# CHONSPQX/modulated-deform-conv

Hardware: AMD Instinct MI355X
Metric: fwd+bwd GSamples/s, MDCN2d 3x3 C=256 56x56 B=32; %HBM roofline (higher is better)
Workload: dtype f32; 1 GPU; ModulatedDeformConv2d 3x3, C_in=C_out=256, 56x56, deformable_group=1, fp32, B=32 per GPU, forward+backward (BASELINE.json configs[1]); global_batch=32, parallelism=dp1 batch-sharded

## Files before the change

### modulated_deform_conv_amd/csrc/mfma_bwd_data.hip

```cpp
#include "mfma_kernels.hpp"
#include "mfma_tile.hpp"
#include <algorithm>
#include <map>
#include <mutex>
#include <stdio.h>
#include <stdlib.h>

namespace mdconv {

namespace {

int grid_for(int64_t total) {
  int64_t b = (total + 255) / 256;
  return (int)(b > 8192 ? 8192 : (b < 1 ? 1 : b));
}

__device__ __forceinline__ void pack_wq_items(const Geom &g, int ochunks, int cblks, const float *__restrict__ w,
                                              float *__restrict__ wq, int64_t first, int64_t step) {
  const int64_t total = (int64_t)g.K * ochunks * cblks * 2 * 64;
  for (int64_t i = first; i < total; i += step) {
    int64_t r = i;
    const int lane = (int)(r & 63); r >>= 6;
    const int q = (int)(r & 1); r >>= 1;
    const int cblk = (int)(r % cblks); r /= cblks;
// ... 6 lines not shown
    for (int s = 0; s < 4; ++s) {
      const int o = ob + s;
      v[s] = (o < g.O && c < g.C && o / g.Og == c / g.Cg)
                 ? w[((int64_t)o * g.Cg + (c % g.Cg)) * g.K + tap] : 0.f;
    }
    reinterpret_cast<float4 *>(wq)[i] = make_float4(v[0], v[1], v[2], v[3]);
  }
}

__global__ __launch_bounds__(256) void pack_wq_kernel(Geom g, int ochunks, int cblks,
                                                      const float *__restrict__ w,
                                                      float *__restrict__ wq) {
  pack_wq_items(g, ochunks, cblks, w, wq, (int64_t)blockIdx.x * 256 + threadIdx.x, (int64_t)gridDim.x * 256);
}

__global__ __launch_bounds__(256) void bwd_prep_kernel(Geom g, int ochunks, int cblks, const float *__restrict__ w,
                                                       float *__restrict__ wq, int *__restrict__ cnt, int64_t cnt_n,
                                                       const float *__restrict__ x, float *__restrict__ xt,
                                                       int nb_pack, int nb_zero, int qtiles, int ctiles) {
  __shared__ float t[32][33];
  int bid = blockIdx.x;
  if (bid < nb_pack) {
    pack_wq_items(g, ochunks, cblks, w, wq, (int64_t)bid * 256 + threadIdx.x, (int64_t)nb_pack * 256);
    return;
  }
  bid -= nb_pack;
  if (bid < nb_zero) {
    for (int64_t i = (int64_t)bid * 256 + threadIdx.x; i < cnt_n; i += (int64_t)nb_zero * 256) cnt[i] = 0;
    return;
  }
  bid -= nb_zero;
  const int qx = bid % qtiles, cy = (bid / qtiles) % ctiles, b = bid / (qtiles * ctiles);
  nchw_to_nhwc_tile(t, g.C, g.S_i, x, xt, b, cy * 32, qx * 32);
}



template <int ND, bool MOD, int WAVES_C, int QPQ, bool CL>
__global__ __launch_bounds__(256, 2) void mfma_bwd_data_kernel(
    Geom g, BwdDims bd, const float *__restrict__ input, const float *__restrict__ gout,
    const float *__restrict__ wq, const float *__restrict__ offset, const float *__restrict__ mask,
    float *__restrict__ gcol, float *__restrict__ grad_offset, float *__restrict__ grad_mask,
    float *__restrict__ ga, float *__restrict__ bias_part, int *__restrict__ cnt,
    int *__restrict__ table, const float *__restrict__ xt, int ntiles, int n_full, int n_tail, int tpw) {
  constexpr int NC = 1 << ND, NP = NC / 2;
  constexpr int MB = 2;
  constexpr int WAVES_P = 4 / WAVES_C;
  constexpr int BNP = 32 * WAVES_P;
  constexpr int RB = ND == 2 ? 8 : 4;
  constexpr int NBATCH = MB * 16 / RB;
  constexpr int HS = NBATCH / 2, CPS = NC / HS;
  constexpr int kOob = 0x7ffffff0;
  extern __shared__ __attribute__((aligned(16))) float smem[];
  const int T_o = bd.ochunks;
  const int gpitch = T_o * 16 + 4;
  float *Gs = smem;
  float *red = smem + BNP * gpitch;
  const int kTapGroup = bd.tap_group;

  const int tid = threadIdx.x, lane = tid & 63, kh = lane >> 5;
  const int wave = __builtin_amdgcn_readfirstlane(tid >> 6);
  const int wc = wave / WAVES_P, wp = wave % WAVES_P;

  int u0, u1;
  if ((int)blockIdx.x < n_full) {
    u0 = xcd_remap(blockIdx.x, n_full) * g.K * tpw;
    u1 = u0 + g.K * tpw;
  } else {
    const int j = xcd_remap(blockIdx.x - n_full, n_tail);
    const int64_t tail_units = (int64_t)(ntiles - n_full * tpw) * g.K;
    u0 = n_full * tpw * g.K + (int)(tail_units * j / n_tail);
    u1 = n_full * tpw * g.K + (int)(tail_units * (j + 1) / n_tail);
  }
  if (u0 >= u1) return;

  const int passes = bd.cblks_q / (2 * WAVES_C);
  const int iters = (u1 - u0) * passes;
// ... 37 lines not shown
#pragma unroll
      for (int q = 0; q < 2; ++q)
        ra[i][q] = buf_load4(r_wq, a_lane + (i * 2 + q) * frag_bytes, soff);
  };
  float4 ra0[MB][2], ra1[MB][2], ra2[MB][2], ra3[MB][2];
  {
    int q_lo, q_n;
    krange(0, q_lo, q_n);
    a_cur = a_base(u0 % g.K, 0, q_lo);
    n_cur = 4;
    load_a(ra0, a_off(0));
    load_a(ra1, a_off(1));
    load_a(ra2, a_off(2));
  }

  struct Pix { int n0, b, pix; bool live; int oc[ND]; };
  auto pix_of_tile = [&](int tile, Pix &px) {
    px.n0 = tile * BNP;
    const int n_raw = px.n0 + wp * 32 + (lane & 31);
    px.live = n_raw < g.N;
    const int n_l = px.live ? n_raw : g.N - 1;
    px.b = n_l / g.S_o;
    px.pix = n_l - px.b * g.S_o;
    out_coords<ND>(g, px.pix, px.oc);
  };
  Pix pc, pp;
  pix_of_tile(u0 / g.K, pc);
  pp = pc;

  auto load_gout_tile = [&](int tile) {
    const int j = tid % BNP, osub = tid / BNP;
    constexpr int OSTEP = 256 / BNP;
    const int n_t = min(tile * BNP + j, g.N - 1);
    const int b_t = n_t / g.S_o, pix_t = n_t - b_t * g.S_o;
    const bool t_live = tile * BNP + j < g.N;
    const float *src = gout + ((int64_t)b_t * g.O) * g.S_o + pix_t;
    float *dst = Gs + j * gpitch;
    const int Opad = T_o * 16;
#pragma unroll 8
// ... 78 lines not shown
  for (int pi = 0; pi < NP; ++pi) voff[pi] = kOob;
#pragma unroll
  for (int ci = 0; ci < NC; ++ci) voffc[ci] = kOob;
#pragma unroll
  for (int ci = 0; ci < NC; ++ci) S[ci] = 0.f;
#pragma unroll
  for (int a = 0; a < ND; ++a) delta_n[a] = 0.f;
#pragma unroll
  for (int a = 0; a < ND - 1; ++a) fac.ol[a] = fac.oh[a] = fac.osl[a] = fac.osh[a] = 0.f;
  fac.xw = fac.yw = fac.xs = fac.ys = 0.f;
#pragma unroll
  for (int i = 0; i < MB; ++i)
#pragma unroll
    for (int r = 0; r < 16; ++r) accp[i][r] = 0.f;

  auto new_tap_state = [&](int tapp, int dgp, bool count) {
    int tcd[ND];
    tap_coords<ND>(g, tapp, tcd);
    TapCoef<ND, float> tc;
    make_tap<ND, float>(g, pp.oc, tcd, delta_n, true, tc);
    mg = (!g.range_gate || tc.inside) ? m_n : 0.f;
    int pidx[NP];
    float px[NP], py[NP];
    make_pairs<ND, float>(g, tc, 1.f, pidx, px, py);
    bool prx[NP], pry[NP];
    make_pairs_read<ND, float>(g, tc, prx, pry);
    if (ND == 3 && count && kh == 0 && pp.live) {
      SampleAnchor<ND> sa;
      sample_anchor<ND>(g, tc, 1.f, sa);
      if (sa.on) atomicAdd(cnt + ((int64_t)pp.b * g.DG + dgp) * bd.S_e + sa.qa, 1);
    }
    if (ND == 2 && count && kh == 0 && pp.live) {
      int aidx[NP];
      float ax[NP], ay[NP];
      make_pairs_f<ND, float>(g, tc, tc.wl, tc.wha, 1.f, aidx, ax, ay);
      int *cseg = cnt + ((int64_t)pp.b * g.DG + dgp) * g.S_i;
#pragma unroll
      for (int pi = 0; pi < NP; ++pi)
        if (ax[pi] != 0.f || ay[pi] != 0.f) atomicAdd(cseg + aidx[pi], 1);
    }
    if (count && kh == 0) {
      const int n = pp.n0 + wp * 32 + lane;
      if (n < bd.Np) {
        int *e = table + ((int64_t)(dgp * g.K + tapp) * bd.Np + n) * (2 * NC);
        int ev[2 * NC];
#pragma unroll
        for (int pi = 0; pi < NP; ++pi) {
          if (bd.cl) {
            ev[2 * pi] = pp.live && prx[pi] ? (pp.b * g.S_i + pidx[pi]) * g.C * 4 : kOob;
            ev[2 * pi + 1] = pp.live && pry[pi] ? (pp.b * g.S_i + pidx[pi] + 1) * g.C * 4 : kOob;
          } else {
            ev[pi] = !pp.live ? 0
                     : ((prx[pi] || pry[pi]) ? ((pp.b * g.C * g.S_i + pidx[pi]) * 4) | (pry[pi] && !prx[pi] ? 1 : 0) | (prx[pi] && !pry[pi] ? 2 : 0)
                                             : kOob);
            ev[NP + pi] = 0;
          }
          ev[NC + 2 * pi] = pp.live ? __float_as_int(px[pi] * m_n) : 0;
          ev[NC + 2 * pi + 1] = pp.live ? __float_as_int(py[pi] * m_n) : 0;
        }
#pragma unroll
        for (int q4 = 0; q4 < 2 * NC; q4 += 4)
          *reinterpret_cast<int4 *>(e + q4) = make_int4(ev[q4], ev[q4 + 1], ev[q4 + 2], ev[q4 + 3]);
      }
    }
#pragma unroll
    for (int pi = 0; pi < NP; ++pi) {
      voff[pi] = (prx[pi] || pry[pi]) ? (pp.b * g.C * g.S_i + pidx[pi] + 4 * kh * g.S_i) * 4 : kOob;
      if (!CL) {
        bad[2 * pi] = __ballot(pry[pi] && !prx[pi]);
        bad[2 * pi + 1] = __ballot(prx[pi] && !pry[pi]);
      }
      voffc[2 * pi] = prx[pi] ? (pp.b * g.S_i + pidx[pi]) * g.C * 4 + 16 * kh : kOob;
      voffc[2 * pi + 1] = pry[pi] ? (pp.b * g.S_i + pidx[pi] + 1) * g.C * 4 + 16 * kh : kOob;
    }
    {
      constexpr int L = ND - 1;
      const int lc = tc.last_lc, hc = tc.last_lc + tc.delta[L];
      const int cl = min(lc, g.in_sz[L] - 2);
      fac.xw = (lc == cl ? tc.wl[L] : 0.f) + (hc == cl ? tc.wh[L] : 0.f);
      fac.yw = (lc == cl + 1 ? tc.wl[L] : 0.f) + (hc == cl + 1 ? tc.wh[L] : 0.f);
      fac.xs = (lc == cl ? tc.sl[L] : 0.f) + (hc == cl ? tc.sh[L] : 0.f);
      fac.ys = (lc == cl + 1 ? tc.sl[L] : 0.f) + (hc == cl + 1 ? tc.sh[L] : 0.f);
#pragma unroll
      for (int a = 0; a < L; ++a) { fac.ol[a] = tc.wl[a]; fac.oh[a] = tc.wh[a]; fac.osl[a] = tc.sl[a]; fac.osh[a] = tc.sh[a]; }
    }
    gc_voff = pp.live ? ((((pp.b * g.K + tapp) * g.S_o + pp.pix) * g.C) + 4 * kh) * 4 : kOob;
    if (CL && kh == 0) {
      int *st = St + lane * kStRow;
#pragma unroll
      for (int c4 = 0; c4 < NC; c4 += 4)
        *reinterpret_cast<int4 *>(st + c4) = make_int4(voffc[c4], voffc[c4 + 1], voffc[c4 + 2], voffc[c4 + 3]);
      st[NC] = gc_voff;
    }
#pragma unroll
    for (int ci = 0; ci < NC; ++ci) S[ci] = 0.f;
  };

  struct Batch { float f[RB * NC]; };
  auto gather = [&](int q, int cbase_p, Batch &v) {
    const int mb = (q * RB) / 16, r0 = (q * RB) % 16;
    if (CL) {
// ... 130 lines not shown
      const int pix = lane & 31, swz = pk_swz(pix);
      float *dst = Pk + pix * 64;
#pragma unroll
      for (int i = 0; i < MB; ++i)
#pragma unroll
        for (int rq = 0; rq < 4; ++rq)
          *reinterpret_cast<float4 *>(dst + 4 * ((i * 8 + 2 * rq + kh) ^ swz)) =
              make_float4(acc[i][4 * rq], acc[i][4 * rq + 1], acc[i][4 * rq + 2], acc[i][4 * rq + 3]);
    } else {
#pragma unroll
      for (int i = 0; i < MB; ++i) accp[i] = acc[i];
    }
  };

  int grp_lo = (u0 % g.K) % kTapGroup;
  auto finish_tap = [&](int tapp, int blk, bool flush_ok, bool last) {
    float goff[ND], gm = 0.f;
    {
      constexpr int L = ND - 1;
      float Tw[NP], Ts[NP];
#pragma unroll
      for (int pi = 0; pi < NP; ++pi) {
        Tw[pi] = fmaf(fac.xw, S[2 * pi], fac.yw * S[2 * pi + 1]);
        Ts[pi] = fmaf(fac.xs, S[2 * pi], fac.ys * S[2 * pi + 1]);
      }
#pragma unroll
      for (int a = 0; a < ND; ++a) goff[a] = 0.f;
#pragma unroll
      for (int pi = 0; pi < NP; ++pi) {
        float ow = 1.f;
#pragma unroll
// ... 7 lines not shown
          for (int a2 = 0; a2 < L; ++a2) {
            const bool hi = (pi >> (L - 1 - a2)) & 1;
            od *= (a2 == a) ? (hi ? fac.osh[a2] : fac.osl[a2]) : (hi ? fac.oh[a2] : fac.ol[a2]);
          }
          goff[a] = fmaf(od, Tw[pi], goff[a]);
        }
      }
#pragma unroll
      for (int a = 0; a < ND; ++a) goff[a] *= mg;
    }
    if (!CL) {
#pragma unroll
      for (int a = 0; a < ND; ++a) goff[a] += __shfl_xor(goff[a], 32, 64);
      gm += __shfl_xor(gm, 32, 64);
    }
    if (bd.red_floats == 0) {
      if (kh == 0 && pp.live) {
        const int64_t ob = ((int64_t)pp.b * (ND * g.K) + ND * tapp) * g.S_o + pp.pix;
#pragma unroll
        for (int a = 0; a < ND; ++a) {
          float *dst = grad_offset + ob + (int64_t)a * g.S_o;
          *dst = g.acc_data ? *dst + goff[a] : goff[a];
        }
        if (MOD) {
          float *dst = grad_mask + ((int64_t)pp.b * g.K + tapp) * g.S_o + pp.pix;
          *dst = g.acc_data ? *dst + gm : gm;
        }
      }
      return;
    }
    const int slot = tapp % kTapGroup;
    if (kh == 0) {
      float *rp = red + ((slot * nblk + blk) * (ND + 1)) * BNP + wp * 32 + lane;
#pragma unroll
      for (int a = 0; a < ND; ++a) rp[a * BNP] = goff[a];
      rp[ND * BNP] = gm;
    }
    if (flush_ok && (slot == kTapGroup - 1 || tapp == g.K - 1 || last)) {
      __syncthreads();
      const int tap0 = tapp - slot;
      const int per_slot = g.DG * (ND + 1) * BNP;
      const int items = (slot + 1 - grp_lo) * per_slot;
      for (int x = tid; x < items; x += 256) {
        const int jj = x % BNP, a = (x / BNP) % (ND + 1), dgi = (x / (BNP * (ND + 1))) % g.DG;
        const int sl = grp_lo + x / per_slot;
        const int n = pp.n0 + jj;
        if (n < g.N && (MOD || a < ND)) {
          float sum = 0.f;
          for (int y = 0; y < bpd; ++y)
            sum += red[((sl * nblk + dgi * bpd + y) * (ND + 1) + a) * BNP + jj];
          const int b = n / g.S_o, pix = n - b * g.S_o, tp = tap0 + sl;
          const int64_t seg = (int64_t)b * g.DG + dgi;
          float *dst = a < ND ? grad_offset + (seg * (ND * g.K) + ND * tp + a) * g.S_o + pix
                              : grad_mask + (seg * g.K + tp) * g.S_o + pix;
          *dst = g.acc_data ? *dst + sum : sum;
        }
      }
      __syncthreads();
      grp_lo = 0;
    }
  };

  auto mma = [&](const float4 (&ra)[MB][2], const float *bp, bool fresh) {
    const float4 b0 = *reinterpret_cast<const float4 *>(bp);
    const float4 b1 = *reinterpret_cast<const float4 *>(bp + 8);
    const f32x16 zero = {0.f, 0.f, 0.f, 0.f, 0.f, 0.f, 0.f, 0.f, 0.f, 0.f, 0.f, 0.f, 0.f, 0.f, 0.f, 0.f};
#pragma unroll
    for (int q = 0; q < 2; ++q)
#pragma unroll
// ... 16 lines not shown
    __builtin_amdgcn_sched_barrier(0);
    mma(ra1, bq + (t + 1) * 16, false);
    load_a(ra1, a_off(t + 5));
    __builtin_amdgcn_sched_barrier(0);
    mma(ra2, bq + (t + 2) * 16, false);
    load_a(ra2, a_off(t + 6));
    __builtin_amdgcn_sched_barrier(0);
    mma(ra3, bq + (t + 3) * 16, false);
  };
  auto quad = [&](int t, bool fresh) { quad_head(t); quad_tail(t, fresh); };

  int tile_c = -1;
  int tapp = 0, passp = 0;
  int tile = u0 / g.K, tap = u0 - tile * g.K, pass = 0;
  for (int it = 0; it < iters; ++it) {
    if (it > 0 && (passp == 0 || per_block)) {
      const int blk = passp * WAVES_C + wc;
      if (per_block) new_tap_state(tapp, min(blk * 64, g.C - 1) / g.Cdg, blk % bpd == 0 && blk * 64 < g.C);
      else new_tap_state(tapp, 0, wc == 0);
    }
    if (tile != tile_c) {
      if (tile_c >= 0) __syncthreads();
      if (gout_vec) load_gout_tile_vec(tile);
      else load_gout_tile(tile);
      pix_of_tile(tile, pc);
      tile_c = tile;
      __syncthreads();
      if (tap == 0 && pass == 0) emit_ga(tile);
    }
    if (pass == 0 || per_block) {
      const int dg = per_block ? min((pass * WAVES_C + wc) * 64, g.C - 1) / g.Cdg : 0;
      const int64_t seg = (int64_t)pc.b * g.DG + dg;
      const int64_t ob = (seg * (ND * g.K) + ND * tap) * g.S_o + pc.pix;
#pragma unroll
      for (int a = 0; a < ND; ++a) delta_n[a] = offset[ob + (int64_t)a * g.S_o];
      if (MOD) m_n = mask[(seg * g.K + tap) * g.S_o + pc.pix];
    }
    int nq;
    {
      int q_lo, tn = tap, pn = pass + 1;
      krange(pass, q_lo, nq);
      a_cur = a_base(tap, pass, q_lo);
      n_cur = nq * 4;
      b_cur = q_lo * 64;
      if (pn == passes) { pn = 0; tn = tap + 1 == g.K ? 0 : tap + 1; }
      int q_lo2, nq2;
      krange(pn, q_lo2, nq2);
      a_nxt = a_base(tn, pn, q_lo2);
    }
    const int cbase_p = (passp * WAVES_C + wc) * 64;
    if (QPQ == 0) {
// ... 12 lines not shown
      __builtin_amdgcn_sched_barrier(0);
      if (QPQ > 0) {
        quad_tail(q * QPQ * 4, q == 0);
#pragma unroll
        for (int jq = 1; jq < QPQ; ++jq) quad((q * QPQ + jq) * 4, false);
      } else {
        for (int qd = nq * q / NBATCH; qd < nq * (q + 1) / NBATCH; ++qd) quad(qd * 4, false);
      }
      __builtin_amdgcn_sched_barrier(0);
      consume(q, cbase_p, v);
      asm volatile("" ::: "memory");
      __builtin_amdgcn_sched_barrier(0);
    }
    collect();
    if (it > 0 && (passp == passes - 1 || per_block))
      finish_tap(tapp, per_block ? passp * WAVES_C + wc : wc, passp == passes - 1, false);
    park();
    pp = pc;
    tapp = tap;
    passp = pass;
    if (++pass == passes) {
      pass = 0;
      if (++tap == g.K) { tap = 0; ++tile; }
    }
  }
  {
    if (passp == 0 || per_block) {
      const int blk = passp * WAVES_C + wc;
      if (per_block) new_tap_state(tapp, min(blk * 64, g.C - 1) / g.Cdg, blk % bpd == 0 && blk * 64 < g.C);
      else new_tap_state(tapp, 0, wc == 0);
    }
    const int cbase_p = (passp * WAVES_C + wc) * 64;
    static_assert(NBATCH % 2 == 0, "pairs of drain batches");
#pragma unroll
    for (int q = 0; q < NBATCH; q += 2) {
      Batch v0, v1;
      gather(q, cbase_p, v0);
      gather(q + 1, cbase_p, v1);
      asm volatile("" ::: "memory");
      __builtin_amdgcn_sched_barrier(0);
      consume(q, cbase_p, v0);
      consume(q + 1, cbase_p, v1);
      asm volatile("" ::: "memory");
      __builtin_amdgcn_sched_barrier(0);
    }
    collect();
    finish_tap(tapp, per_block ? passp * WAVES_C + wc : wc, true, true);
  }
}


template <int ND, bool MOD>
__global__ __launch_bounds__(256) void csr_fill_kernel(Geom g, const float *__restrict__ offset,
                                                       const float *__restrict__ mask,
                                                       int *__restrict__ cursor,
                                                       const int *__restrict__ rowptr,
                                                       int4 *__restrict__ entries) {
  constexpr int NP = 1 << (ND - 1);
  const int64_t total = (int64_t)g.B * g.DG * g.K * g.S_o;
  for (int64_t i = (int64_t)blockIdx.x * 256 + threadIdx.x; i < total; i += (int64_t)gridDim.x * 256) {
    const int pix = (int)(i % g.S_o);
    const int tap = (int)((i / g.S_o) % g.K);
// ... 31 lines not shown
__global__ __launch_bounds__(256) void csr_scan_kernel(int S, const int *__restrict__ cnt,
                                            int *__restrict__ rowptr) {
  csr_scan_chunk(S, cnt, rowptr);
}

}

int pack_wq_f32(const Geom &g, const BwdDims &bd, const float *weight, float *wq, hipStream_t stream) {
  const int64_t total = (int64_t)g.K * bd.ochunks * bd.cblks_q * 2 * 64;
  hipLaunchKernelGGL(pack_wq_kernel, dim3(grid_for(total)), dim3(256), 0, stream, g, bd.ochunks,
                     bd.cblks_q, weight, wq);
  return check_launch("pack_wq");
}

int bwd_prep_f32(const Geom &g, const BwdDims &bd, const float *weight, float *wq, int *cnt, const float *x,
                 float *xt, hipStream_t stream) {
  const int64_t pack_total = (int64_t)g.K * bd.ochunks * bd.cblks_q * 2 * 64;
  const int64_t cnt_n = (int64_t)g.B * g.DG * bd.S_e;
  int nb_pack = grid_for(pack_total), nb_zero = grid_for(cnt_n);
  if (nb_pack > 512) nb_pack = 512;
  if (nb_zero > 256) nb_zero = 256;
  const int qtiles = (g.S_i + 31) / 32, ctiles = g.C / 32;
  const int64_t nb_t = xt ? (int64_t)qtiles * ctiles * g.B : 0;
  if (nb_t + nb_pack + nb_zero > 0x7fffffff) {
    int rc = pack_wq_f32(g, bd, weight, wq, stream);
    if (!rc) rc = csr_zero_f32(g, bd, cnt, stream);
    if (!rc && xt) rc = nchw_to_nhwc_f32(g, x, xt, stream);
    return rc;
  }
  hipLaunchKernelGGL(bwd_prep_kernel, dim3((unsigned)(nb_pack + nb_zero + nb_t)), dim3(256), 0, stream, g, bd.ochunks,
                     bd.cblks_q, weight, wq, cnt, cnt_n, x, xt, nb_pack, nb_zero, qtiles, ctiles);
  return check_launch("bwd_prep");
}

int num_cus() {
  static int n = 0;
  if (n == 0) {
    int dev = 0, v = 0;
    if (hipGetDevice(&dev) == hipSuccess &&
        hipDeviceGetAttribute(&v, hipDeviceAttributeMultiprocessorCount, dev) == hipSuccess && v > 0)
      n = v;
    else
      n = 256;
  }
  return n;
}

size_t bwd_data_lds_bytes(const Geom &g, const BwdDims &bd) {
  const int bnp = 32 * (4 / bd.waves_c);
  const int passes = bd.cblks_q / (2 * bd.waves_c);
  const size_t red = (size_t)bd.red_floats;
  const size_t cl = bd.cl_drain ? (size_t)4 * 32 * 64 + (size_t)4 * 32 * (2 * (1 << g.nd) + 4) : 0;
  return ((size_t)bnp * (bd.ochunks * 16 + 4) + red + cl) * sizeof(float);
}

int mfma_bwd_data_f32(const Geom &g, const BwdDims &bd, const Tensors &t, const float *wq,
                      float *gcol, float *ga, float *bias_part, int *cnt, int *table,
                      const float *xt, hipStream_t stream) {
#define LAUNCH_BD_(ND, MOD, WC, QPQ, CL)                                                            \
  do {                                                                                          \
    const int bnp = 32 * (4 / WC);                                                              \
    const int ntiles = (g.N + bnp - 1) / bnp;                                                   \
    const size_t lds = bwd_data_lds_bytes(g, bd);                                               \
     \
     \
     \
     \
    static std::once_flag attr_once;                                                            \
    static hipError_t attr_err = hipSuccess;                                                    \
    std::call_once(attr_once, [] {                                                              \
      attr_err = hipFuncSetAttribute((const void *)mfma_bwd_data_kernel<ND, MOD, WC, QPQ, CL>,  \
                                     hipFuncAttributeMaxDynamicSharedMemorySize, (int)kBwdDataLdsCap); \
    });                                                                                         \
// ... 14 lines not shown
        it = occ_by_lds.emplace(lds, nq > 0 ? nq : (lds * 2 <= 160 * 1024 ? 2 : 1)).first;      \
      }                                                                                         \
      occ_q = it->second;                                                                       \
    }                                                                                           \
    const int slots = num_cus() * occ_q;                                                        \
    const int tpw = 2;                        \
    const int n_full = ntiles / (slots * tpw) * slots;                                          \
    static const bool debug_plan = getenv("MDCONV_DEBUG_PLAN") != nullptr;                      \
    if (debug_plan)                                                                             \
      fprintf(stderr, "[mdconv] GEMM-1 plan: %d tiles, %zu B LDS, %d resident per CU\n", ntiles, lds, occ_q); \
    const int n_tail = (int)std::min<int64_t>((int64_t)(ntiles - n_full * tpw) * g.K, slots);   \
    hipLaunchKernelGGL((mfma_bwd_data_kernel<ND, MOD, WC, QPQ, CL>), dim3(n_full + n_tail), \
                       dim3(256), lds, stream,                                                  \
                       g, bd, (const float *)t.input, (const float *)t.grad_output, wq,         \
                       (const float *)t.offset, (const float *)t.mask, gcol,                    \
                       (float *)t.grad_offset, (float *)t.grad_mask, ga, bias_part, cnt, table, xt,        \
                       ntiles, n_full, n_tail, tpw);                                            \
  } while (0)
                                                \
#define LAUNCH_BD(ND, MOD, WC, QPQ)                                                             \
  do {                                                                                          \
    if (xt != nullptr && bd.cl_drain) LAUNCH_BD_(ND, MOD, WC, QPQ, true);                       \
    else LAUNCH_BD_(ND, MOD, WC, QPQ, false);                                                   \
  } while (0)
#define LAUNCH_BD2(ND, MOD)                                                                     \
  do {                                                                                          \
    const int nbatch = ND == 2 ? 4 : 8, nquads = bd.ochunks / 4;                                \
                   \
    const int qpq = (ND == 2 && g.G == 1 && nquads % nbatch == 0 && nquads / nbatch <= 2) ? nquads / nbatch : 0; \
    if (bd.waves_c == 4) {                                                                      \
      if (ND == 2 && qpq == 1) LAUNCH_BD(ND, MOD, 4, (ND == 2 ? 1 : 0));                        \
// ... 38 lines not shown
```

### modulated_deform_conv_amd/csrc/mfma_kernels.hip

```cpp
#include "mfma_plan.hpp"

#include <stdio.h>
#include <stdlib.h>

#include <atomic>
#include <mutex>
#include <vector>

namespace mdconv {

namespace {

__global__ __launch_bounds__(256) void pack_weights_kernel(Geom g, PackDims pd,
                                                           const float *__restrict__ w,
                                                           float *__restrict__ wp,
                                                           float *__restrict__ wq) {
  const int64_t total = (int64_t)g.G * g.K * pd.Cgp * pd.Ogp;
  const int mblks = pd.Ogp / 32, cchunks = pd.Cgp / kBK;
  for (int64_t i = (int64_t)blockIdx.x * 256 + threadIdx.x; i < total; i += (int64_t)gridDim.x * 256) {
    int64_t r = i;
    const int s = (int)(r & 3); r >>= 2;
    const int lane = (int)(r & 63); r >>= 6;
    const int q = (int)(r & 1); r >>= 1;
    const int mblk = (int)(r % mblks); r /= mblks;
// ... 104 lines not shown
  bd.sample_keyed = g.nd == 3 ? 1 : 0;
  bd.S_e = bd.sample_keyed ? hp_anchor_space(g) : g.S_i;
  bd.off_cnt = off;  off += align_up((size_t)g.B * g.DG * bd.S_e * sizeof(int));
  bd.off_rowptr = off; off += skip.input ? 0 : align_up((size_t)g.B * g.DG * (bd.S_e + 1) * sizeof(int));
  bd.off_entries = off; off += skip.input ? 0 : align_up((size_t)g.B * g.DG * g.K * g.S_o * (bd.sample_keyed ? 32 : (nc / 2) * 16));
  bd.bias_tiles = (g.N + 32 * (4 / bd.waves_c) - 1) / (32 * (4 / bd.waves_c));
  bd.off_bias = off; off += align_up((size_t)bd.bias_tiles * g.O * sizeof(float));
  bd.off_xt = off;   off += bd.cl ? align_up((size_t)g.B * g.S_i * g.C * sizeof(float)) : 0;
  static const int c2i_env = getenv("MDCONV_C2I3D") ? atoi(getenv("MDCONV_C2I3D")) : 2;
  bd.two_pass = bd.sample_keyed && c2i_env >= 2 ? 1 : 0;
  bd.off_sums = off; off += bd.two_pass && !skip.input ? align_up(col2im3d_sums_bytes(g)) : 0;
  bd.off_bstage = off; off += g.with_bias && !skip.weight ? align_up(grad_bias_stage_bytes(g)) : 0;
  bd.off_sort = off;
  off += g.det && !skip.input ? align_up(csr_sort_scratch_bytes(bd.sample_keyed ? 2 : 1, (int64_t)g.K * g.S_o * (bd.sample_keyed ? 1 : nc / 2),
                                                 g.B * g.DG)) : 0;
  bd.off_end = off;
  return bd;
}

namespace {

constexpr size_t kChunkCeiling = ((size_t)1 << 31) - (1 << 16);

size_t fwd_core_bytes(const Geom &gc) {
  const PackDims pd = pack_dims(gc);
  size_t n = align_up((size_t)gc.G * gc.K * pd.Cgp * pd.Ogp * sizeof(float));
  if (fwd_channels_last(gc)) n += align_up(fwd_cl_bytes(gc));
  n += align_up(fwd_tail_bytes(gc));
  return n;
}
// ... 83 lines not shown
bool bwd_fork_enabled() { return bwd_fork_mode() != 0; }

int backward_chunk_f32(const Geom &g, const BwdDims &bd, const Tensors &t, char *base, hipStream_t stream,
                       bool weights_final, Skip skip) {
  float *wq = (float *)(base + bd.off_wq);
  float *ga = (float *)(base + bd.off_ga);
  int *table = (int *)(base + bd.off_table);
  float *part = (float *)(base + bd.off_part);
  float *gcol = (float *)(base + bd.off_gcol);
  int *cnt = (int *)(base + bd.off_cnt), *rowptr = (int *)(base + bd.off_rowptr);
  void *entries = base + bd.off_entries;
  int rc;
  float *bias_part = g.with_bias ? (float *)(base + bd.off_bias) : nullptr;
  float *bstage = g.with_bias ? (float *)(base + bd.off_bstage) : nullptr;
  float *xt = bd.cl ? (float *)(base + bd.off_xt) : nullptr;
  if ((rc = bwd_prep_f32(g, bd, (const float *)t.weight, wq, cnt, (const float *)t.input, xt, stream))) return rc;
  profile_mark(1, true, stream, "mfma_bwd_data_kernel");
  rc = mfma_bwd_data_f32(g, bd, t, wq, gcol, ga, bias_part, cnt, table, xt, stream);
  profile_mark(1, false, stream);
  if (rc) return rc;
  Fork fk;
  const bool fork = !skip.input && !skip.weight && bwd_fork_enabled() && get_fork(stream, &fk);
  hipStream_t gs = stream;
  auto gemm2 = [&](bool bias_here) {
    int r = mfma_bwd_weight_f32(g, bd, t, ga, table, part, bias_part, xt, stream);
    if (!r && bias_here) r = grad_bias_f32(g, bd, bias_part, bstage, (float *)t.grad_bias, stream);
    if (!r && !bias_here && g.with_bias && hipStreamWaitEvent(stream, fk.bias, 0) != hipSuccess) {
      set_error("backward fork failed");
      r = MDCONV_ELAUNCH;
    }
    if (!r && weights_final) r = record_weight_ready(stream);
    return r;
  };
// ... 182 lines not shown
```

### modulated_deform_conv_amd/csrc/mfma_tile.hpp

```cpp
#pragma once
#include "mdconv_common.hpp"

namespace mdconv {

typedef float f32x16 __attribute__((ext_vector_type(16)));

constexpr int kBK = 16;

struct PackDims {
  int Cgp;
  int Ogp;
  int BM;
};

inline PackDims pack_dims(const Geom &g) {
  PackDims pd;
  pd.BM = g.Og > 128 ? 256 : (g.Og > 64 ? 128 : 64);
  pd.Cgp = (g.Cg + 2 * kBK - 1) / (2 * kBK) * (2 * kBK);
  pd.Ogp = (g.Og + pd.BM - 1) / pd.BM * pd.BM;
  return pd;
}

__device__ __forceinline__ int xcd_remap(int bid, int n) {
  const int q = n >> 3, r = n & 7;
// ... 36 lines not shown
  int wtile;
  int OgpB, mblks, mtiles;
  int Cp, cblks;
  int splits, pairs_per_split;
  int ochunks;
  int waves_c, cblks_q;
  int bias_tiles;
  int red_floats;
  int tap_group;
  int cl_drain;
  int sample_keyed;
  int S_e;
  size_t off_wq, off_ga, off_table, off_part, off_gcol, off_cnt, off_rowptr, off_entries, off_bias,
      off_xt, off_sums, off_bstage, off_sort, off_end;
  int two_pass;
};
BwdDims bwd_dims(const Geom &g, Skip skip = Skip());

#ifdef __HIPCC__
__device__ __forceinline__ void nchw_to_nhwc_tile(float (*t)[33], int C, int S, const float *__restrict__ x,
                                                  float *__restrict__ xt, int b, int c0, int q0) {
  const int tx = threadIdx.x & 31, ty = threadIdx.x >> 5;
  const float *src = x + ((size_t)b * C + c0) * S;
  float *dst = xt + ((size_t)b * S + q0) * C + c0;
#pragma unroll
  for (int r = ty; r < 32; r += 8) t[r][tx] = (q0 + tx < S) ? src[(size_t)r * S + q0 + tx] : 0.f;
  __syncthreads();
#pragma unroll
  for (int r = ty; r < 32; r += 8)
    if (q0 + r < S) dst[(size_t)r * C + tx] = t[tx][r];
}
// ... 12 lines not shown
size_t fwd_cl_bytes(const Geom &g);
int mfma_forward_cl_f32(const Geom &g, const PackDims &pd, const Tensors &t, const float *wp, float *part,
                        float *xt, hipStream_t stream);
int mfma_bwd_weight_f32(const Geom &g, const BwdDims &bd, const Tensors &t, const float *ga,
                        const int *table, float *part, const float *bias_part, const float *xt,
                        hipStream_t stream);
int mfma_bwd_weight_cl_launch(const Geom &g, const BwdDims &bd, const float *xt, const float *ga,
                              const int *table, float *part, hipStream_t stream);
int mfma_bwd_weight_cl_occupancy(int nd, bool padn, int wtile);
int mfma_bwd_weight_occupancy(int nd, bool padn, int wtile);
int device_cus();
bool bwd_channels_last(const Geom &g);
int nchw_to_nhwc_f32(const Geom &g, const float *x, float *xt, hipStream_t stream);
int pack_wq_f32(const Geom &g, const BwdDims &bd, const float *weight, float *wq, hipStream_t stream);
int bwd_prep_f32(const Geom &g, const BwdDims &bd, const float *weight, float *wq, int *cnt, const float *x,
                 float *xt, hipStream_t stream);
size_t grad_bias_stage_bytes(const Geom &g);
int grad_bias_f32(const Geom &g, const BwdDims &bd, const float *bias_part, float *stage, float *grad_bias,
                  hipStream_t stream);
size_t bwd_data_lds_bytes(const Geom &g, const BwdDims &bd);
constexpr size_t kBwdDataLdsCap = 150 * 1024;
int mfma_bwd_data_f32(const Geom &g, const BwdDims &bd, const Tensors &t, const float *wq,
                      float *gcol, float *ga, float *bias_part, int *cnt, int *table,
                      const float *xt, hipStream_t stream);
int csr_zero_f32(const Geom &g, const BwdDims &bd, int *cnt, hipStream_t stream);
int csr_build_f32(const Geom &g, const BwdDims &bd, const Tensors &t, int *cnt, int *rowptr,
                  void *entries, hipStream_t stream);
int col2im_f32(const Geom &g, const BwdDims &bd, const Tensors &t, const float *gcol,
               const int *rowptr, const void *entries, float *sums, hipStream_t stream);
int csr_fill3d_f32(const Geom &g, const BwdDims &bd, const Tensors &t, int *cursor,
                   const int *rowptr, void *entries, hipStream_t stream);
int col2im3d_f32(const Geom &g, const BwdDims &bd, const Tensors &t, const float *gcol,
                 const int *rowptr, const void *entries, float *sums, hipStream_t stream);
size_t col2im3d_sums_bytes(const Geom &g);

}
```

Measured before the change: 73.01 GSamples/s.

## Precompute per-tap index records loaded as scalar constants in bwd-data kernel

Adds a small per-tap record table (tap offsets, gcol/mask row bases, slot/flush flags, strides), built in an extra block of the prep kernel. The backward-data kernel reads each record through a constant address space pointer, so the loads can be scalar, instead of recomputing tap coordinates and 64-bit index math each iteration. Per-pixel bases are also precomputed once per tile, and addressing moves to 32-bit byte offsets. The cost is an extra global table and a dependency on it, and 32-bit offsets risk overflow on large tensors. The finish_tap direct-write path is also restricted to WAVES_C==1.

```diff
diff --git a/modulated_deform_conv_amd/csrc/mfma_bwd_data.hip b/modulated_deform_conv_amd/csrc/mfma_bwd_data.hip
--- a/modulated_deform_conv_amd/csrc/mfma_bwd_data.hip
+++ b/modulated_deform_conv_amd/csrc/mfma_bwd_data.hip
@@ -44,12 +44,64 @@
   pack_wq_items(g, ochunks, cblks, w, wq, (int64_t)blockIdx.x * 256 + threadIdx.x, (int64_t)gridDim.x * 256);
 }
 
+enum TapRec {
+  TR_TP = 0,
+  TR_GCOL = 3,
+  TR_MROW = 4,
+  TR_TAB = 5,
+  TR_SLOT = 6,
+  TR_FLUSH = 7,
+  TR_IN = 8,
+  TR_FLAGS = 11,
+  TR_C4 = 12,
+  TR_TABDG = 13,
+  TR_SI = 14,
+  TR_SE = 15,
+};
+typedef int i32x16 __attribute__((ext_vector_type(16)));
+typedef const __attribute__((address_space(4))) i32x16 *krec_p;
+template <typename T> __device__ __forceinline__ T *at32(T *base, int idx) {
+  return (T *)((char *)base + (size_t)((unsigned)idx * (unsigned)sizeof(T)));
+}
+__device__ __forceinline__ void tap_rec_items(const Geom &g, int Np, int S_e, int tap_group, int *__restrict__ trec) {
+  for (int tap = threadIdx.x; tap < g.K; tap += 256) {
+    int r[kTapRecInts];
+    int tc[3] = {0, 0, 0};
+    if (g.nd == 2) tap_coords<2>(g, tap, tc); else tap_coords<3>(g, tap, tc);
+    for (int a = 0; a < 3; ++a) {
+      r[TR_TP + a] = a < g.nd ? tc[a] * g.dil[a] - g.pad[a] : 0;
+      r[TR_IN + a] = a < g.nd ? g.in_sz[a] : 1;
+    }
+    const int slot = tap % tap_group;
+    r[TR_GCOL] = tap * g.S_o * g.C * 4;
+    r[TR_MROW] = tap * g.S_o;
+    r[TR_TAB] = tap * Np * (2 << g.nd);
+    r[TR_SLOT] = slot;
+    r[TR_FLUSH] = (slot == tap_group - 1 || tap == g.K - 1) ? 1 : 0;
+    r[TR_FLAGS] = (g.load_eps ? 1 : 0) | (g.atom_eps ? 2 : 0) | (g.range_gate ? 4 : 0);
+    r[TR_C4] = g.C * 4;
+    r[TR_TABDG] = g.K * Np * (2 << g.nd);
+    r[TR_SI] = g.S_i;
+    r[TR_SE] = S_e;
+    for (int i = 0; i < kTapRecInts; ++i) trec[tap * kTapRecInts + i] = r[i];
+  }
+}
+__global__ __launch_bounds__(256) void tap_rec_kernel(Geom g, int Np, int S_e, int tap_group, int *__restrict__ trec) {
+  tap_rec_items(g, Np, S_e, tap_group, trec);
+}
+
 __global__ __launch_bounds__(256) void bwd_prep_kernel(Geom g, int ochunks, int cblks, const float *__restrict__ w,
                                                        float *__restrict__ wq, int *__restrict__ cnt, int64_t cnt_n,
                                                        const float *__restrict__ x, float *__restrict__ xt,
-                                                       int nb_pack, int nb_zero, int qtiles, int ctiles) {
+                                                       int nb_pack, int nb_zero, int qtiles, int ctiles,
+                                                       int *__restrict__ trec, int Np, int S_e, int tap_group) {
   __shared__ float t[32][33];
   int bid = blockIdx.x;
+  if (bid == 0) {
+    tap_rec_items(g, Np, S_e, tap_group, trec);
+    return;
+  }
+  bid -= 1;
   if (bid < nb_pack) {
     pack_wq_items(g, ochunks, cblks, w, wq, (int64_t)bid * 256 + threadIdx.x, (int64_t)nb_pack * 256);
     return;
@@ -72,7 +124,8 @@
     const float *__restrict__ wq, const float *__restrict__ offset, const float *__restrict__ mask,
     float *__restrict__ gcol, float *__restrict__ grad_offset, float *__restrict__ grad_mask,
     float *__restrict__ ga, float *__restrict__ bias_part, int *__restrict__ cnt,
-    int *__restrict__ table, const float *__restrict__ xt, int ntiles, int n_full, int n_tail, int tpw) {
+    int *__restrict__ table, const float *__restrict__ xt, const int *__restrict__ trec_g, int ntiles, int n_full,
+    int n_tail, int tpw) {
   constexpr int NC = 1 << ND, NP = NC / 2;
   constexpr int MB = 2;
   constexpr int WAVES_P = 4 / WAVES_C;
@@ -91,6 +144,7 @@
   const int tid = threadIdx.x, lane = tid & 63, kh = lane >> 5;
   const int wave = __builtin_amdgcn_readfirstlane(tid >> 6);
   const int wc = wave / WAVES_P, wp = wave % WAVES_P;
+  const krec_p trec = (krec_p)trec_g;
 
   int u0, u1;
   if ((int)blockIdx.x < n_full) {
@@ -158,7 +212,7 @@
     load_a(ra2, a_off(2));
   }
 
-  struct Pix { int n0, b, pix; bool live; int oc[ND]; };
+  struct Pix { int n0, b, pix; bool live; int os[ND], bsi, gc0, mrow; };
   auto pix_of_tile = [&](int tile, Pix &px) {
     px.n0 = tile * BNP;
     const int n_raw = px.n0 + wp * 32 + (lane & 31);
@@ -166,7 +220,13 @@
     const int n_l = px.live ? n_raw : g.N - 1;
     px.b = n_l / g.S_o;
     px.pix = n_l - px.b * g.S_o;
-    out_coords<ND>(g, px.pix, px.oc);
+    int oc[ND];
+    out_coords<ND>(g, px.pix, oc);
+#pragma unroll
+    for (int a = 0; a < ND; ++a) px.os[a] = oc[a] * g.stride[a];
+    px.bsi = px.b * g.S_i;
+    px.gc0 = ((px.b * g.K * g.S_o + px.pix) * g.C + 4 * kh) * 4;
+    px.mrow = px.b * g.DG * g.K * g.S_o + px.pix;
   };
   Pix pc, pp;
   pix_of_tile(u0 / g.K, pc);
@@ -275,44 +335,56 @@
 #pragma unroll
     for (int r = 0; r < 16; ++r) accp[i][r] = 0.f;
 
-  auto new_tap_state = [&](int tapp, int dgp, bool count) {
+  auto new_tap_state = [&](const i32x16 &rec, int dgp, bool count) {
+    Geom gs;
     int tcd[ND];
-    tap_coords<ND>(g, tapp, tcd);
+#pragma unroll
+    for (int a = 0; a < ND; ++a) {
+      tcd[a] = rec[TR_TP + a];
+      gs.in_sz[a] = rec[TR_IN + a];
+      gs.stride[a] = 1;
+      gs.pad[a] = 0;
+      gs.dil[a] = 1;
+    }
+    gs.load_eps = rec[TR_FLAGS] & 1;
+    gs.atom_eps = rec[TR_FLAGS] & 2;
+    gs.range_gate = rec[TR_FLAGS] & 4;
+    const int C4 = rec[TR_C4];
     TapCoef<ND, float> tc;
-    make_tap<ND, float>(g, pp.oc, tcd, delta_n, true, tc);
-    mg = (!g.range_gate || tc.inside) ? m_n : 0.f;
+    make_tap<ND, float>(gs, pp.os, tcd, delta_n, true, tc);
+    mg = (!gs.range_gate || tc.inside) ? m_n : 0.f;
     int pidx[NP];
     float px[NP], py[NP];
-    make_pairs<ND, float>(g, tc, 1.f, pidx, px, py);
+    make_pairs<ND, float>(gs, tc, 1.f, pidx, px, py);
     bool prx[NP], pry[NP];
-    make_pairs_read<ND, float>(g, tc, prx, pry);
+    make_pairs_read<ND, float>(gs, tc, prx, pry);
     if (ND == 3 && count && kh == 0 && pp.live) {
       SampleAnchor<ND> sa;
-      sample_anchor<ND>(g, tc, 1.f, sa);
-      if (sa.on) atomicAdd(cnt + ((int64_t)pp.b * g.DG + dgp) * bd.S_e + sa.qa, 1);
+      sample_anchor<ND>(gs, tc, 1.f, sa);
+      if (sa.on) atomicAdd(at32(cnt, (pp.b * g.DG + dgp) * rec[TR_SE] + sa.qa), 1);
     }
     if (ND == 2 && count && kh == 0 && pp.live) {
       int aidx[NP];
       float ax[NP], ay[NP];
-      make_pairs_f<ND, float>(g, tc, tc.wl, tc.wha, 1.f, aidx, ax, ay);
-      int *cseg = cnt + ((int64_t)pp.b * g.DG + dgp) * g.S_i;
+      make_pairs_f<ND, float>(gs, tc, tc.wl, tc.wha, 1.f, aidx, ax, ay);
+      const int cseg = pp.bsi * g.DG + dgp * rec[TR_SI];
 #pragma unroll
       for (int pi = 0; pi < NP; ++pi)
-        if (ax[pi] != 0.f || ay[pi] != 0.f) atomicAdd(cseg + aidx[pi], 1);
+        if (ax[pi] != 0.f || ay[pi] != 0.f) atomicAdd(at32(cnt, cseg + aidx[pi]), 1);
     }
     if (count && kh == 0) {
       const int n = pp.n0 + wp * 32 + lane;
       if (n < bd.Np) {
-        int *e = table + ((int64_t)(dgp * g.K + tapp) * bd.Np + n) * (2 * NC);
+        int *e = at32(table, rec[TR_TAB] + dgp * rec[TR_TABDG] + n * (2 * NC));
         int ev[2 * NC];
 #pragma unroll
         for (int pi = 0; pi < NP; ++pi) {
           if (bd.cl) {
-            ev[2 * pi] = pp.live && prx[pi] ? (pp.b * g.S_i + pidx[pi]) * g.C * 4 : kOob;
-            ev[2 * pi + 1] = pp.live && pry[pi] ? (pp.b * g.S_i + pidx[pi] + 1) * g.C * 4 : kOob;
+            ev[2 * pi] = pp.live && prx[pi] ? (pp.bsi + pidx[pi]) * C4 : kOob;
+            ev[2 * pi + 1] = pp.live && pry[pi] ? (pp.bsi + pidx[pi] + 1) * C4 : kOob;
           } else {
             ev[pi] = !pp.live ? 0
-                     : ((prx[pi] || pry[pi]) ? ((pp.b * g.C * g.S_i + pidx[pi]) * 4) | (pry[pi] && !prx[pi] ? 1 : 0) | (prx[pi] && !pry[pi] ? 2 : 0)
+                     : ((prx[pi] || pry[pi]) ? (pp.bsi * C4 + pidx[pi] * 4) | (pry[pi] && !prx[pi] ? 1 : 0) | (prx[pi] && !pry[pi] ? 2 : 0)
                                              : kOob);
             ev[NP + pi] = 0;
           }
@@ -326,18 +398,18 @@
     }
 #pragma unroll
     for (int pi = 0; pi < NP; ++pi) {
-      voff[pi] = (prx[pi] || pry[pi]) ? (pp.b * g.C * g.S_i + pidx[pi] + 4 * kh * g.S_i) * 4 : kOob;
+      voff[pi] = (prx[pi] || pry[pi]) ? pp.bsi * C4 + (pidx[pi] + 4 * kh * rec[TR_SI]) * 4 : kOob;
       if (!CL) {
         bad[2 * pi] = __ballot(pry[pi] && !prx[pi]);
         bad[2 * pi + 1] = __ballot(prx[pi] && !pry[pi]);
       }
-      voffc[2 * pi] = prx[pi] ? (pp.b * g.S_i + pidx[pi]) * g.C * 4 + 16 * kh : kOob;
-      voffc[2 * pi + 1] = pry[pi] ? (pp.b * g.S_i + pidx[pi] + 1) * g.C * 4 + 16 * kh : kOob;
+      voffc[2 * pi] = prx[pi] ? (pp.bsi + pidx[pi]) * C4 + 16 * kh : kOob;
+      voffc[2 * pi + 1] = pry[pi] ? (pp.bsi + pidx[pi] + 1) * C4 + 16 * kh : kOob;
     }
     {
       constexpr int L = ND - 1;
       const int lc = tc.last_lc, hc = tc.last_lc + tc.delta[L];
-      const int cl = min(lc, g.in_sz[L] - 2);
+      const int cl = min(lc, gs.in_sz[L] - 2);
       fac.xw = (lc == cl ? tc.wl[L] : 0.f) + (hc == cl ? tc.wh[L] : 0.f);
       fac.yw = (lc == cl + 1 ? tc.wl[L] : 0.f) + (hc == cl + 1 ? tc.wh[L] : 0.f);
       fac.xs = (lc == cl ? tc.sl[L] : 0.f) + (hc == cl ? tc.sh[L] : 0.f);
@@ -345,7 +417,7 @@
 #pragma unroll
       for (int a = 0; a < L; ++a) { fac.ol[a] = tc.wl[a]; fac.oh[a] = tc.wh[a]; fac.osl[a] = tc.sl[a]; fac.osh[a] = tc.sh[a]; }
     }
-    gc_voff = pp.live ? ((((pp.b * g.K + tapp) * g.S_o + pp.pix) * g.C) + 4 * kh) * 4 : kOob;
+    gc_voff = pp.live ? pp.gc0 + rec[TR_GCOL] : kOob;
     if (CL && kh == 0) {
       int *st = St + lane * kStRow;
 #pragma unroll
@@ -506,7 +578,7 @@
   };
 
   int grp_lo = (u0 % g.K) % kTapGroup;
-  auto finish_tap = [&](int tapp, int blk, bool flush_ok, bool last) {
+  auto finish_tap = [&](int tapp, const i32x16 &rec, int blk, bool flush_ok, bool last) {
     float goff[ND], gm = 0.f;
     {
       constexpr int L = ND - 1;
@@ -544,7 +616,7 @@
       for (int a = 0; a < ND; ++a) goff[a] += __shfl_xor(goff[a], 32, 64);
       gm += __shfl_xor(gm, 32, 64);
     }
-    if (bd.red_floats == 0) {
+    if (WAVES_C == 1 && bd.red_floats == 0) {
       if (kh == 0 && pp.live) {
         const int64_t ob = ((int64_t)pp.b * (ND * g.K) + ND * tapp) * g.S_o + pp.pix;
 #pragma unroll
@@ -559,30 +631,33 @@
       }
       return;
     }
-    const int slot = tapp % kTapGroup;
+    const int slot = rec[TR_SLOT];
     if (kh == 0) {
       float *rp = red + ((slot * nblk + blk) * (ND + 1)) * BNP + wp * 32 + lane;
 #pragma unroll
       for (int a = 0; a < ND; ++a) rp[a * BNP] = goff[a];
       rp[ND * BNP] = gm;
     }
-    if (flush_ok && (slot == kTapGroup - 1 || tapp == g.K - 1 || last)) {
+    if (flush_ok && (rec[TR_FLUSH] || last)) {
       __syncthreads();
       const int tap0 = tapp - slot;
       const int per_slot = g.DG * (ND + 1) * BNP;
       const int items = (slot + 1 - grp_lo) * per_slot;
+      const int jj = tid % BNP;
+      const int n = pp.n0 + jj;
+      const int b = min(n, g.N - 1) / g.S_o, pix = n - b * g.S_o;
       for (int x = tid; x < items; x += 256) {
-        const int jj = x % BNP, a = (x / BNP) % (ND + 1), dgi = (x / (BNP * (ND + 1))) % g.DG;
-        const int sl = grp_lo + x / per_slot;
-        const int n = pp.n0 + jj;
+        const int z = x / (BNP * (ND + 1)), a = (x / BNP) % (ND + 1);
+        const int zs = g.DG == 1 ? z : z / g.DG, dgi = z - zs * g.DG;
+        const int sl = grp_lo + zs;
         if (n < g.N && (MOD || a < ND)) {
           float sum = 0.f;
           for (int y = 0; y < bpd; ++y)
             sum += red[((sl * nblk + dgi * bpd + y) * (ND + 1) + a) * BNP + jj];
-          const int b = n / g.S_o, pix = n - b * g.S_o, tp = tap0 + sl;
-          const int64_t seg = (int64_t)b * g.DG + dgi;
-          float *dst = a < ND ? grad_offset + (seg * (ND * g.K) + ND * tp + a) * g.S_o + pix
-                              : grad_mask + (seg * g.K + tp) * g.S_o + pix;
+          const int tp = tap0 + sl;
+          const int seg = b * g.DG + dgi;
+          float *dst = a < ND ? at32(grad_offset, (seg * (ND * g.K) + ND * tp + a) * g.S_o + pix)
+                              : at32(grad_mask, (seg * g.K + tp) * g.S_o + pix);
           *dst = g.acc_data ? *dst + sum : sum;
         }
       }
@@ -629,10 +704,11 @@
   int tapp = 0, passp = 0;
   int tile = u0 / g.K, tap = u0 - tile * g.K, pass = 0;
   for (int it = 0; it < iters; ++it) {
+    const i32x16 recp = trec[tapp];
     if (it > 0 && (passp == 0 || per_block)) {
       const int blk = passp * WAVES_C + wc;
-      if (per_block) new_tap_state(tapp, min(blk * 64, g.C - 1) / g.Cdg, blk % bpd == 0 && blk * 64 < g.C);
-      else new_tap_state(tapp, 0, wc == 0);
+      if (per_block) new_tap_state(recp, min(blk * 64, g.C - 1) / g.Cdg, blk % bpd == 0 && blk * 64 < g.C);
+      else new_tap_state(recp, 0, wc == 0);
     }
     if (tile != tile_c) {
       if (tile_c >= 0) __syncthreads();
@@ -645,11 +721,12 @@
     }
     if (pass == 0 || per_block) {
       const int dg = per_block ? min((pass * WAVES_C + wc) * 64, g.C - 1) / g.Cdg : 0;
-      const int64_t seg = (int64_t)pc.b * g.DG + dg;
-      const int64_t ob = (seg * (ND * g.K) + ND * tap) * g.S_o + pc.pix;
-#pragma unroll
-      for (int a = 0; a < ND; ++a) delta_n[a] = offset[ob + (int64_t)a * g.S_o];
-      if (MOD) m_n = mask[(seg * g.K + tap) * g.S_o + pc.pix];
+      const int srow = (per_block ? dg * g.K * g.S_o : 0) + trec[tap][TR_MROW];
+      const int mi = pc.mrow + srow;
+      const int oi = ND * (mi - pc.pix) + pc.pix;
+#pragma unroll
+      for (int a = 0; a < ND; ++a) delta_n[a] = *at32(offset + (int64_t)a * g.S_o, oi);
+      if (MOD) m_n = *at32(mask, mi);
     }
     int nq;
     {
@@ -692,7 +769,7 @@
     }
     collect();
     if (it > 0 && (passp == passes - 1 || per_block))
-      finish_tap(tapp, per_block ? passp * WAVES_C + wc : wc, passp == passes - 1, false);
+      finish_tap(tapp, recp, per_block ? passp * WAVES_C + wc : wc, passp == passes - 1, false);
     park();
     pp = pc;
     tapp = tap;
@@ -703,10 +780,11 @@
     }
   }
   {
+    const i32x16 recp = trec[tapp];
     if (passp == 0 || per_block) {
       const int blk = passp * WAVES_C + wc;
-      if (per_block) new_tap_state(tapp, min(blk * 64, g.C - 1) / g.Cdg, blk % bpd == 0 && blk * 64 < g.C);
-      else new_tap_state(tapp, 0, wc == 0);
+      if (per_block) new_tap_state(recp, min(blk * 64, g.C - 1) / g.Cdg, blk % bpd == 0 && blk * 64 < g.C);
+      else new_tap_state(recp, 0, wc == 0);
     }
     const int cbase_p = (passp * WAVES_C + wc) * 64;
     static_assert(NBATCH % 2 == 0, "pairs of drain batches");
@@ -723,7 +801,7 @@
       __builtin_amdgcn_sched_barrier(0);
     }
     collect();
-    finish_tap(tapp, per_block ? passp * WAVES_C + wc : wc, true, true);
+    finish_tap(tapp, recp, per_block ? passp * WAVES_C + wc : wc, true, true);
   }
 }
 
@@ -785,7 +863,7 @@
 }
 
 int bwd_prep_f32(const Geom &g, const BwdDims &bd, const float *weight, float *wq, int *cnt, const float *x,
-                 float *xt, hipStream_t stream) {
+                 float *xt, int *trec, hipStream_t stream) {
   const int64_t pack_total = (int64_t)g.K * bd.ochunks * bd.cblks_q * 2 * 64;
   const int64_t cnt_n = (int64_t)g.B * g.DG * bd.S_e;
   int nb_pack = grid_for(pack_total), nb_zero = grid_for(cnt_n);
@@ -793,14 +871,19 @@
   if (nb_zero > 256) nb_zero = 256;
   const int qtiles = (g.S_i + 31) / 32, ctiles = g.C / 32;
   const int64_t nb_t = xt ? (int64_t)qtiles * ctiles * g.B : 0;
-  if (nb_t + nb_pack + nb_zero > 0x7fffffff) {
+  if (nb_t + nb_pack + nb_zero + 1 > 0x7fffffff) {
     int rc = pack_wq_f32(g, bd, weight, wq, stream);
     if (!rc) rc = csr_zero_f32(g, bd, cnt, stream);
     if (!rc && xt) rc = nchw_to_nhwc_f32(g, x, xt, stream);
+    if (!rc) {
+      hipLaunchKernelGGL(tap_rec_kernel, dim3(1), dim3(256), 0, stream, g, bd.Np, bd.S_e, bd.tap_group, trec);
+      rc = check_launch("tap_rec");
+    }
     return rc;
   }
-  hipLaunchKernelGGL(bwd_prep_kernel, dim3((unsigned)(nb_pack + nb_zero + nb_t)), dim3(256), 0, stream, g, bd.ochunks,
-                     bd.cblks_q, weight, wq, cnt, cnt_n, x, xt, nb_pack, nb_zero, qtiles, ctiles);
+  hipLaunchKernelGGL(bwd_prep_kernel, dim3((unsigned)(1 + nb_pack + nb_zero + nb_t)), dim3(256), 0, stream, g, bd.ochunks,
+                     bd.cblks_q, weight, wq, cnt, cnt_n, x, xt, nb_pack, nb_zero, qtiles, ctiles, trec, bd.Np, bd.S_e,
+                     bd.tap_group);
   return check_launch("bwd_prep");
 }
 
@@ -827,7 +910,7 @@
 
 int mfma_bwd_data_f32(const Geom &g, const BwdDims &bd, const Tensors &t, const float *wq,
                       float *gcol, float *ga, float *bias_part, int *cnt, int *table,
-                      const float *xt, hipStream_t stream) {
+                      const float *xt, const int *trec, hipStream_t stream) {
 #define LAUNCH_BD_(ND, MOD, WC, QPQ, CL)                                                            \
   do {                                                                                          \
     const int bnp = 32 * (4 / WC);                                                              \
@@ -872,7 +955,7 @@
                        dim3(256), lds, stream,                                                  \
                        g, bd, (const float *)t.input, (const float *)t.grad_output, wq,         \
                        (const float *)t.offset, (const float *)t.mask, gcol,                    \
-                       (float *)t.grad_offset, (float *)t.grad_mask, ga, bias_part, cnt, table, xt,        \
+                       (float *)t.grad_offset, (float *)t.grad_mask, ga, bias_part, cnt, table, xt, trec,  \
                        ntiles, n_full, n_tail, tpw);                                            \
   } while (0)
                                                 \
diff --git a/modulated_deform_conv_amd/csrc/mfma_kernels.hip b/modulated_deform_conv_amd/csrc/mfma_kernels.hip
--- a/modulated_deform_conv_amd/csrc/mfma_kernels.hip
+++ b/modulated_deform_conv_amd/csrc/mfma_kernels.hip
@@ -142,6 +142,7 @@
   bd.off_sort = off;
   off += g.det && !skip.input ? align_up(csr_sort_scratch_bytes(bd.sample_keyed ? 2 : 1, (int64_t)g.K * g.S_o * (bd.sample_keyed ? 1 : nc / 2),
                                                  g.B * g.DG)) : 0;
+  bd.off_trec = off; off += align_up((size_t)g.K * kTapRecInts * sizeof(int));
   bd.off_end = off;
   return bd;
 }
@@ -255,9 +256,10 @@
   float *bias_part = g.with_bias ? (float *)(base + bd.off_bias) : nullptr;
   float *bstage = g.with_bias ? (float *)(base + bd.off_bstage) : nullptr;
   float *xt = bd.cl ? (float *)(base + bd.off_xt) : nullptr;
-  if ((rc = bwd_prep_f32(g, bd, (const float *)t.weight, wq, cnt, (const float *)t.input, xt, stream))) return rc;
+  int *trec = (int *)(base + bd.off_trec);
+  if ((rc = bwd_prep_f32(g, bd, (const float *)t.weight, wq, cnt, (const float *)t.input, xt, trec, stream))) return rc;
   profile_mark(1, true, stream, "mfma_bwd_data_kernel");
-  rc = mfma_bwd_data_f32(g, bd, t, wq, gcol, ga, bias_part, cnt, table, xt, stream);
+  rc = mfma_bwd_data_f32(g, bd, t, wq, gcol, ga, bias_part, cnt, table, xt, trec, stream);
   profile_mark(1, false, stream);
   if (rc) return rc;
   Fork fk;
diff --git a/modulated_deform_conv_amd/csrc/mfma_tile.hpp b/modulated_deform_conv_amd/csrc/mfma_tile.hpp
--- a/modulated_deform_conv_amd/csrc/mfma_tile.hpp
+++ b/modulated_deform_conv_amd/csrc/mfma_tile.hpp
@@ -74,7 +74,9 @@
   size_t off_wq, off_ga, off_table, off_part, off_gcol, off_cnt, off_rowptr, off_entries, off_bias,
       off_xt, off_sums, off_bstage, off_sort, off_end;
   int two_pass;
+  size_t off_trec;
 };
+constexpr int kTapRecInts = 16;
 BwdDims bwd_dims(const Geom &g, Skip skip = Skip());
 
 #ifdef __HIPCC__
@@ -117,7 +119,7 @@
 int nchw_to_nhwc_f32(const Geom &g, const float *x, float *xt, hipStream_t stream);
 int pack_wq_f32(const Geom &g, const BwdDims &bd, const float *weight, float *wq, hipStream_t stream);
 int bwd_prep_f32(const Geom &g, const BwdDims &bd, const float *weight, float *wq, int *cnt, const float *x,
-                 float *xt, hipStream_t stream);
+                 float *xt, int *trec, hipStream_t stream);
 size_t grad_bias_stage_bytes(const Geom &g);
 int grad_bias_f32(const Geom &g, const BwdDims &bd, const float *bias_part, float *stage, float *grad_bias,
                   hipStream_t stream);
@@ -125,7 +127,7 @@
 constexpr size_t kBwdDataLdsCap = 150 * 1024;
 int mfma_bwd_data_f32(const Geom &g, const BwdDims &bd, const Tensors &t, const float *wq,
                       float *gcol, float *ga, float *bias_part, int *cnt, int *table,
-                      const float *xt, hipStream_t stream);
+                      const float *xt, const int *trec, hipStream_t stream);
 int csr_zero_f32(const Geom &g, const BwdDims &bd, int *cnt, hipStream_t stream);
 int csr_build_f32(const Geom &g, const BwdDims &bd, const Tensors &t, int *cnt, int *rowptr,
                   void *entries, hipStream_t stream);
```

Result: no change. 73.46 GSamples/s (median of 6 runs) (+0.6%).
